# SutirthaChakraborty/RTFS-Net

Hardware: AMD Instinct MI355X
Metric: mixtures/sec forward (2 s@16 kHz, 2-spk) RTFS-Net-4 (higher is better)
Workload: dtype f32 (f16x3 split-precision MFMA products, f32 accumulate; every tensor in HBM is f32)

## Files before the change

rtfs-net_amd/csrc/api.hip:

```cpp
#include "api_common.h"
#include <atomic>
#include <vector>

namespace {

struct Cursor {
    const float* p;
    size_t off = 0;
    explicit Cursor(const float* base) : p(base) {}
    const float* take(size_t n) {
        const float* r = p ? p + off : nullptr;
        off += (n + 63) / 64 * 64;
        return r;
    }
};

struct Fork {
    hipStream_t st = nullptr;
    RtfsSide side{};
    bool open = false;
    int begin(hipStream_t owner, int slot) {
        st = owner;
        CHECK(rtfs_side_stream(owner, slot, &side));
        if (hipEventRecord(side.fork, st) != hipSuccess || hipStreamWaitEvent(side.stream, side.fork, 0) != hipSuccess) return RTFS_ERR_LAUNCH;
// ... 198 lines not shown
    a.w16_ct = reinterpret_cast<const half8*>(p.w16_ct);
    a.wf_l0 = reinterpret_cast<const half8*>(p.wf_l0);
    a.wf_l = reinterpret_cast<const half8*>(p.wf_l);
    a.wf_ct = reinterpret_cast<const half8*>(p.wf_ct);
    a.wc16 = p.wc16;
    a.bias16 = p.bias16;
    a.bt = p.bt;
    return a;
}

int dualpath(const DpPack& p, const float* x, float* out, int B, int T, int F, int dim, float* tA, float* tB, hipStream_t st) {
    const size_t plane = (size_t)T * F;
    if (dim == 4) {
        RTFS_RETURN_IF(F < 8 || F > 250, RTFS_ERR_SHAPE);
        if (!gemm_f32() && !p.whh) return launch_dualpath16(dp16_args(p, x, out, B * T, T, F, CH * plane, F, plane), st);
        return launch_dualpath(dp_args(p, x, out, T, F, CH * plane, F, plane), B * T, st);
    }
    RTFS_RETURN_IF(T < 8 || T > (p.whh ? 250 : 512), RTFS_ERR_SHAPE);
    CHECK(launch_transpose(x, tA, B * CH, T, F, st));
    if (T > 256 && !p.whh) {
        const int nb = (int)std::min<size_t>((size_t)B, (((size_t)1 << 32) - 1) / (CH * plane * sizeof(float)));
        for (int b0 = 0; b0 < B; b0 += nb) {
            const int n = std::min(nb, B - b0);
            CHECK(launch_dualpath16(dp16_args(p, tA + (size_t)b0 * CH * plane, tB + (size_t)b0 * CH * plane, n * F, F, T, CH * plane, T, plane), st));
        }
    } else if ((!gemm_f32() || T > 250) && !p.whh) {
        CHECK(launch_dualpath16(dp16_args(p, tA, tB, B * F, F, T, CH * plane, T, plane), st));
    } else {
        CHECK(launch_dualpath(dp_args(p, tA, tB, F, T, CH * plane, T, plane), B * F, st));
    }
    return launch_transpose(tB, out, B * CH, F, T, st);
}

int attention(const AttnPack& p, const float* x, float* out, int B, int T, float* q, float* k, float* v, float* o, hipStream_t st) {
    RowCanArgs a;
    a.x = x;
    a.wt = p.qkv_wt;
    a.bias = p.qkv_b;
    a.slope = p.qkv_slope;
    a.gamma = p.qkv_gamma;
    a.beta = p.qkv_beta;
    a.ngroups = 12;
    for (int g = 0; g <= 12; ++g) a.group_start[g] = g <= 8 ? 4 * g : 32 + 16 * (g - 8);
    for (int g = 0; g < 12; ++g)
        for (int o_ = a.group_start[g]; o_ < a.group_start[g + 1]; ++o_) a.group_of[o_] = (unsigned char)g;
    a.T = T;
    a.q = q;
    a.k = k;
    a.v = v;
    CHECK(launch_row_can_qkv(a, B, st));
    AttnArgs c;
    c.q = q;
    c.k = k;
    c.v = v;
    c.out = o;
    c.T = T;
    c.scale = 1.0f / 16.0f;
    CHECK(launch_attn_core(c, B, st));
    RowCanArgs r;
    r.x = o;
    r.wt = p.proj_wt;
    r.bias = p.proj_b;
    r.slope = p.proj_slope;
    r.gamma = p.proj_gamma;
    r.beta = p.proj_beta;
    r.ngroups = 1;
    r.group_start[0] = 0;
    r.group_start[1] = 64;
    r.T = T;
    r.res = x;
    r.out = out;
    return launch_row_can_proj(r, B, st);
}

struct BlockWs {
    float *residual, *x_enc, *c0, *xf0, *expanded;
    float *c1, *p0, *g, *gF, *tA, *tB, *gT, *gA, *q, *k, *v, *o;
    float *E0, *G0, *E1, *G1, *L1, *xf1, *E2, *G2;
    double* stats;
    int Bfull = 0;
    int cs = 0;
    static constexpr int NSTAT = 11;
    enum { S_C0, S_C1, S_E0, S_G0, S_E1, S_G1, S_L1, S_E2, S_G2, S_L0, S_L2 };
    BlockWs(Arena& a, int B, int T, int F, int cs_ = 0) {
        const size_t Pg = (size_t)(T / 2) * (F / 2);
        cs = cs_ ? cs_ : T * F;
        const size_t P = (size_t)cs;
        Bfull = B;
        residual = a.take<float>(B * CA * P);
        x_enc = a.take<float>(B * CH * P);
        c0 = a.take<float>(B * CH * P);
        xf0 = a.take<float>(B * CH * P);
        expanded = a.take<float>(B * CH * P);
        float** gs[] = {&c1, &p0, &g, &gF, &tA, &tB, &gT, &gA, &v, &o, &E0, &G0, &E1, &G1, &L1, &xf1, &E2, &G2};
        for (float** s : gs) *s = a.take<float>(B * CH * Pg);
        q = a.take<float>(B * CH * Pg / 4);
        k = a.take<float>(B * CH * Pg / 4);
        stats = a.take<double>((size_t)NSTAT * B * 2);
    }
    double* st(int slot, int ) const { return stats ? stats + (size_t)slot * Bfull * 2 : nullptr; }
};

int block_head(const BlockPack& p, const float* x, const float* x_res, int B, int T, int F, BlockWs& w, hipStream_t st, const CafArgs* caf, unsigned* ctr = nullptr) {
// ... 35 lines not shown
    if (zero_stats && hipMemsetAsync(w.stats, 0, sizeof(double) * W::NSTAT * w.Bfull * 2, st) != hipSuccess) return RTFS_ERR_LAUNCH;
    {
        DwArgs a;
        a.x = w.x_enc;
        a.w[0] = p.ds0_w;
        a.bias[0] = p.ds0_b;
        a.out[0] = w.c0;
        a.stats_out[0] = w.st(W::S_C0, B);
        a.C = CH; a.H = T; a.W = F; a.TH = TH_A; a.cs = w.cs;
        CHECK(launch_dw_s1(a, 1, false, 0, B, st));
    }
    DwArgs s14;
    s14.x = w.c0;
    s14.in_stats = w.st(W::S_C0, B); s14.in_inv_count = icF; s14.in_gamma = p.ds0_g; s14.in_beta = p.ds0_be;
    s14.C = CH; s14.H = T; s14.W = F; s14.TH = 64; s14.Hg = Tp; s14.Wg = Fp; s14.cs = w.cs;
    s14.w[0] = p.fus0.loc_w;
    s14.stats_out[0] = w.st(W::S_L0, B);
    s14.rev = 1;
    DwArgs s3;
    s3.x = w.c0;
    s3.in_stats = w.st(W::S_C0, B); s3.in_inv_count = icF; s3.in_gamma = p.ds0_g; s3.in_beta = p.ds0_be;
    s3.w[0] = p.ds1_w;
    s3.bias[0] = p.ds1_b;
    s3.out[0] = w.c1;
    s3.out[1] = w.p0;
    s3.stats_out[0] = w.st(W::S_C1, B);
    s3.C = CH; s3.H = T; s3.W = F; s3.Hg = Tp; s3.Wg = Fp; s3.TH = TH_C; s3.cs = w.cs;
    s3.rev = 1;
    {
        const int rc = launch_dw_s2_stats(s3, s14, B, st);
        if (rc != RTFS_OK) return rc == RTFS_ERR_ARG ? RTFS_ERR_SHAPE : rc;
    }
    CHECK(launch_g_form(w.p0, w.c1, w.st(W::S_C1, B), icG, p.ds1_g, p.ds1_be, w.g, B, CH, Pg, st));
    CHECK(dualpath(p.dpF, w.g, w.gF, B, Tp, Fp, 4, w.tA, w.tB, st));
    CHECK(dualpath(p.dpT, w.gF, w.gT, B, Tp, Fp, 3, w.tA, w.tB, st));
    CHECK(attention(p.attn, w.gT, w.gA, B, Tp, w.q, w.k, w.v, w.o, st));
    {
        DwArgs a;
        a.x = w.gA;
        a.w[0] = p.fus0.emb_w; a.w[1] = p.fus0.gate_w; a.w[2] = p.fus1.emb_w; a.w[3] = p.fus1.gate_w;
        a.out[0] = w.E0; a.out[1] = w.G0; a.out[2] = w.E1; a.out[3] = w.G1;
        a.stats_out[0] = w.st(W::S_E0, B); a.stats_out[1] = w.st(W::S_G0, B);
        a.stats_out[2] = w.st(W::S_E1, B); a.stats_out[3] = w.st(W::S_G1, B);
        a.C = CH; a.H = Tp; a.W = Fp; a.TH = TH_G;
        DwArgs l;
        l.x = w.c1;
        l.in_stats = w.st(W::S_C1, B); l.in_inv_count = icG; l.in_gamma = p.ds1_g; l.in_beta = p.ds1_be;
        l.w[0] = p.fus1.loc_w;
        l.out[0] = w.L1;
        l.stats_out[0] = w.st(W::S_L1, B);
        l.C = CH; l.H = Tp; l.W = Fp; l.TH = TH_G;
        const int rc = launch_dw_g3(a, l, B, st);
        if (rc == RTFS_ERR_ARG) {
            CHECK(launch_dw_s1(a, 4, false, 0, B, st));
            CHECK(launch_dw_s1(l, 1, true, 0, B, st));
        } else {
            CHECK(rc);
        }
    }
    {
        DwArgs a;
        a.x = w.L1; a.gate = w.G1; a.emb = w.E1;
        a.in_combine = 1;
        a.loc_stats = w.st(W::S_L1, B); a.gate_stats = w.st(W::S_G1, B); a.emb_stats = w.st(W::S_E1, B);
        a.loc_gamma = p.fus1.loc_g; a.loc_beta = p.fus1.loc_b;
        a.gate_gamma = p.fus1.gate_g; a.gate_beta = p.fus1.gate_b;
        a.emb_gamma = p.fus1.emb_g; a.emb_beta = p.fus1.emb_b;
        a.g_inv_count = icG;
        a.w[0] = p.cat0.emb_w; a.w[1] = p.cat0.gate_w;
// ... 687 lines not shown
```

rtfs-net_amd/csrc/k_attn.hip:

```cpp
#include "common.h"
#include "kernels.h"
#include "pipe_helpers.h"

#define AF 64

#define RCAN_ROWS 8
#define RCAN_LD 72
template <int NOUT>
__global__ __launch_bounds__(256, 2) void row_can_kernel(RowCanArgs a) {
    constexpr int MT = NOUT / 32, MTW = (MT + 1) / 2;
    constexpr int NR = NOUT / 4;
    constexpr float WSC = 256.f, WINV = 1.f / 256.f;
    __shared__ float Ys[NOUT][RCAN_LD];
    __shared__ float bias_s[NOUT], slope_s[NOUT];
    __shared__ float red[8];
    const int T = a.T, b = blockIdx.y;
    const int tid = threadIdx.x, lane = tid & 63, r = lane & 31, h = lane >> 5;
    const int wave = __builtin_amdgcn_readfirstlane(tid >> 6);
    const int nt = wave & 1, mp = wave >> 1;
    for (int o = tid; o < NOUT; o += 256) {
        bias_s[o] = a.bias[o] * WSC;
        slope_s[o] = a.slope[NOUT == 96 ? a.group_of[o] : 0];
    }
    half8 wh[MTW][4], wl[MTW][4];
#pragma unroll
    for (int m = 0; m < MTW; ++m) {
        const int mt = min(mp + 2 * m, MT - 1);
#pragma unroll
        for (int ks = 0; ks < 4; ++ks)
#pragma unroll
            for (int j = 0; j < 8; ++j) {
                const float w = a.wt[(ks * 16 + 8 * h + j) * NOUT + mt * 32 + r] * WSC;
                const _Float16 hi = (_Float16)w;
                wh[m][ks][j] = hi;
                wl[m][ks][j] = (_Float16)(w - (float)hi);
            }
    }
    auto ln_row = [&](int i) -> int {
        if (NOUT == 64) return wave * 16 + i;
        return i < 4 ? 4 * wave + i : i < 8 ? 16 + 4 * wave + (i - 4) : 32 + 16 * wave + (i - 8);
    };
    __shared__ float gam_s[NOUT][AF], bet_s[NOUT][AF];
    for (int i = tid; i < NOUT * AF; i += 256) {
        gam_s[0][i] = a.gamma[i];
        bet_s[0][i] = a.beta[i];
    }
    const int t0 = blockIdx.x * a.rpw;
    const int nrows = min(a.rpw, T - t0);
    const float* __restrict__ X = a.x + (size_t)b * 64 * T * AF + nt * 32 + r;
    const float* __restrict__ RES = NOUT == 64 ? a.res + ((size_t)b * 64 + wave * 16) * T * AF + lane : nullptr;
    float v[4][8];
    float rs[NOUT == 64 ? 16 : 1];
    auto load_x = [&](int t) {
#pragma unroll
        for (int ks = 0; ks < 4; ++ks)
#pragma unroll
            for (int j = 0; j < 8; ++j) v[ks][j] = X[((size_t)(ks * 16 + 8 * h + j) * T + t) * AF];
    };
    load_x(t0);
    __syncthreads();
    for (int rr = 0; rr < nrows; ++rr) {
        const int t = t0 + rr;
        half8 bh[4], bl[4];
#pragma unroll
        for (int ks = 0; ks < 4; ++ks) {
            unsigned hi[4], lo[4];
#pragma unroll
            for (int jp = 0; jp < 4; ++jp) split2(v[ks][2 * jp], v[ks][2 * jp + 1], hi[jp], lo[jp]);
            bh[ks] = __builtin_bit_cast(half8, *reinterpret_cast<f32x4*>(hi));
            bl[ks] = __builtin_bit_cast(half8, *reinterpret_cast<f32x4*>(lo));
        }
        if (NOUT == 64) {
#pragma unroll
            for (int i = 0; i < 16; ++i) rs[i] = RES[((size_t)i * T + t) * AF];
        }
        load_x(min(t + 1, T - 1));
#pragma unroll
        for (int m = 0; m < MTW; ++m) {
            const int mt = mp + 2 * m;
            if (mt < MT) {
                f32x16 acc;
#pragma unroll
                for (int q = 0; q < 16; ++q) acc[q] = bias_s[mt * 32 + (q & 3) + 8 * (q >> 2) + 4 * h];
#pragma unroll
                for (int ks = 0; ks < 4; ++ks) {
                    acc = __builtin_amdgcn_mfma_f32_32x32x16_f16(wh[m][ks], bh[ks], acc, 0, 0, 0);
                    acc = __builtin_amdgcn_mfma_f32_32x32x16_f16(wh[m][ks], bl[ks], acc, 0, 0, 0);
                    acc = __builtin_amdgcn_mfma_f32_32x32x16_f16(wl[m][ks], bh[ks], acc, 0, 0, 0);
                }
#pragma unroll
                for (int q = 0; q < 16; ++q) {
                    const int o = mt * 32 + (q & 3) + 8 * (q >> 2) + 4 * h;
                    Ys[o][nt * 32 + r] = preluf_(acc[q] * WINV, slope_s[o]);
                }
            }
        }
        __syncthreads();
        float y[NR];
#pragma unroll
        for (int i = 0; i < NR; ++i) y[i] = Ys[ln_row(i)][lane];
        if (NOUT == 96) {
#pragma unroll
            for (int g = 0; g < 3; ++g) {
                const int i0 = g == 0 ? 0 : g == 1 ? 4 : 8, gs = g == 2 ? 16 : 4;
                float s = 0.f;
#pragma unroll
                for (int i = 0; i < gs; ++i) s += y[i0 + i];
                const float mean = wave_sum(s) / (float)(gs * AF);
                float vv = 0.f;
#pragma unroll
                for (int i = 0; i < gs; ++i) {
                    y[i0 + i] -= mean;
                    vv = fmaf(y[i0 + i], y[i0 + i], vv);
                }
                const float rstd = 1.0f / sqrtf(wave_sum(vv) / (float)(gs * AF) + RTFS_EPS);
                float* __restrict__ dst = (g == 0 ? a.q : g == 1 ? a.k : a.v) + (((size_t)b * 4 + wave) * T + t) * (gs * AF) + lane;
#pragma unroll
                for (int i = 0; i < gs; ++i) dst[i * AF] = fmaf(y[i0 + i] * rstd, gam_s[ln_row(i0 + i)][lane], bet_s[ln_row(i0 + i)][lane]);
            }
        } else {
            float s = 0.f;
#pragma unroll
            for (int i = 0; i < 16; ++i) s += y[i];
            s = wave_sum(s);
            if (lane == 0) red[wave] = s;
            __syncthreads();
            const float mean = (red[0] + red[1] + red[2] + red[3]) / (float)(64 * AF);
            float vv = 0.f;
#pragma unroll
            for (int i = 0; i < 16; ++i) {
                y[i] -= mean;
                vv = fmaf(y[i], y[i], vv);
            }
            vv = wave_sum(vv);
            if (lane == 0) red[4 + wave] = vv;
            __syncthreads();
            const float rstd = 1.0f / sqrtf((red[4] + red[5] + red[6] + red[7]) / (float)(64 * AF) + RTFS_EPS);
            float* __restrict__ O = a.out + ((size_t)b * 64 + wave * 16) * T * AF + lane;
#pragma unroll
            for (int i = 0; i < 16; ++i) O[((size_t)i * T + t) * AF] = fmaf(y[i] * rstd, gam_s[ln_row(i)][lane], bet_s[ln_row(i)][lane]) + rs[i];
        }
        __syncthreads();
    }
}

#define ATT_PSC 4096.f
__device__ __forceinline__ void split8(const float (&v)[8], float sc, half8& hi, half8& lo) {
    unsigned h[4], l[4];
#pragma unroll
    for (int jp = 0; jp < 4; ++jp) split2(v[2 * jp] * sc, v[2 * jp + 1] * sc, h[jp], l[jp]);
    hi = __builtin_bit_cast(half8, *reinterpret_cast<f32x4*>(h));
    lo = __builtin_bit_cast(half8, *reinterpret_cast<f32x4*>(l));
}
__global__ __launch_bounds__(256) void attn_core_kernel(AttnArgs a) {
    extern __shared__ __attribute__((aligned(16))) float S[];
    const int T = a.T;
    const int NKT = (T + 31) >> 5;
    const int NK = NKT * 32;
    const int ldp = NK + 4;
    const int tid = threadIdx.x, lane = tid & 63, r = lane & 31, h = lane >> 5;
    const int wave = __builtin_amdgcn_readfirstlane(tid >> 6);
    const int nqt = (T + 31) >> 5;
    const int slot = blockIdx.x >> 3;
    const int pair = (slot / nqt) * 8 + (blockIdx.x & 7);
    if (pair >= a.npairs) return;
    const int q0 = (slot % nqt) * 32, hd = pair & 3, b = pair >> 2;
    const float* __restrict__ Q = a.q + ((size_t)b * 4 + hd) * T * 256;
    const float* __restrict__ K = a.k + ((size_t)b * 4 + hd) * T * 256;
    const float* __restrict__ V = a.v + ((size_t)b * 4 + hd) * T * 1024;

    for (int kg = 0; kg < NKT; kg += 8) {
// ... 89 lines not shown
        for (int ks = 0; ks < nks; ks += 2) {
            load_v(ks + 1, vv[1]);
            step(ks, vv[0]);
            load_v(min(ks + 2, nks - 1), vv[0]);
            step(ks + 1, vv[1]);
        }
        {
            const int c = col0 >> 6, f = col0 & 63;
#pragma unroll
            for (int q = 0; q < 16; ++q) {
                const int qq = q0 + (q & 3) + 8 * (q >> 2) + 4 * h;
                if (qq < T)
                    *reinterpret_cast<f32x4*>(a.out + (((size_t)b * 64 + hd * 16 + c) * T + qq) * AF + f) =
                        f32x4{o[0][q], o[1][q], o[2][q], o[3][q]} * (1.f / ATT_PSC);
            }
        }
    }
}

size_t attn_core_lds_bytes(int T) {
    const int NK = ((T + 31) >> 5) * 32;
    return (size_t)32 * (NK + 4) * sizeof(float);
}

static int rcan_rows(int T, int B) {
    if ((long)T * B >= 3500) return RCAN_ROWS;
    const int r = (int)((long)T * B / 512);
    return r < 1 ? 1 : (r > RCAN_ROWS ? RCAN_ROWS : r);
}
int launch_row_can_qkv(const RowCanArgs& a_, int B, hipStream_t st) {
    RowCanArgs a = a_;
    a.rpw = rcan_rows(a.T, B);
    if (a.ngroups != 12 || a.group_start[8] != 32 || a.group_start[12] != 96) return RTFS_ERR_SHAPE;
    hipLaunchKernelGGL(row_can_kernel<96>, dim3(cdiv(a.T, a.rpw), B), dim3(256), 0, st, a);
    return rtfs_launch_status();
}
int launch_row_can_proj(const RowCanArgs& a_, int B, hipStream_t st) {
    RowCanArgs a = a_;
    a.rpw = rcan_rows(a.T, B);
    if (a.ngroups != 1) return RTFS_ERR_SHAPE;
    hipLaunchKernelGGL(row_can_kernel<64>, dim3(cdiv(a.T, a.rpw), B), dim3(256), 0, st, a);
    return rtfs_launch_status();
}
int launch_attn_core(const AttnArgs& a, int B, hipStream_t st) {
    if (a.T < 1 || a.T > 512) return RTFS_ERR_SHAPE;
    const size_t lds = attn_core_lds_bytes(a.T);
    if (rtfs_set_max_lds((const void*)attn_core_kernel, lds) != RTFS_OK) return RTFS_ERR_LAUNCH;
    AttnArgs a2 = a;
    a2.npairs = B * 4;
    hipLaunchKernelGGL(attn_core_kernel, dim3(cdiv(a2.npairs, 8) * 8 * cdiv(a.T, 32)), dim3(256), lds, st, a2);
    return rtfs_launch_status();
}
```

rtfs-net_amd/csrc/k_dualpath16.hip:

```cpp
#include "common.h"
#include "kernels.h"
#include <stdlib.h>
#include <type_traits>


#define HLD 72
#define WLD 40
#define CLD 72
#define WINV (1.0f / 256.0f)

namespace {

__device__ __forceinline__ void split8(const float (&v)[8], half8& hi, half8& lo) {
#pragma unroll
    for (int i = 0; i < 8; ++i) {
        const _Float16 hh = (_Float16)v[i];
        hi[i] = hh;
        lo[i] = (_Float16)(v[i] - (float)hh);
    }
}

__device__ __forceinline__ float sig2(float z) { return __builtin_amdgcn_rcpf(1.0f + __builtin_amdgcn_exp2f(z)); }

__device__ __forceinline__ float take_half(float v, int ph) {
// ... 322 lines not shown
                        const int co = cot * 32 + (q & 3) + 8 * (q >> 2) + 4 * h;
                        a.out[base + (size_t)co * a.cstride + p] = fmaf(acc[t][q], WINV, res[t][q]);
                    }
                }
            }
        }
        stamp();
    }
}

size_t dp16_lds_bytes(int Ls, int nseq_per_wg) {
    return (size_t)2 * nseq_per_wg * (Ls + 1) * HLD * 2 + (size_t)2 * 2 * 256 * WLD * 2 + (size_t)nseq_per_wg * 2 * 32 * 4;
}

template <int NSEQ, int NHALF, bool PAIRED>
static int launch_dp16_stamp_t(const Dp16Args& a, hipStream_t st) {
    const size_t lds = dp16_lds_bytes(a.Ls, NSEQ);
    if (hipFuncSetAttribute((const void*)dp16_kernel<NSEQ, NHALF, PAIRED, true>, hipFuncAttributeMaxDynamicSharedMemorySize, (int)lds) != hipSuccess)
        return RTFS_ERR_LAUNCH;
    hipLaunchKernelGGL((dp16_kernel<NSEQ, NHALF, PAIRED, true>), dim3(cdiv(a.nseq, NSEQ)), dim3(512), lds, st, a);
    return rtfs_launch_status();
}

template <int NSEQ, int NHALF, bool PAIRED>
static int launch_dp16_t(const Dp16Args& a, hipStream_t st) {
    const size_t lds = dp16_lds_bytes(a.Ls, NSEQ);
    if (rtfs_set_max_lds((const void*)dp16_kernel<NSEQ, NHALF, PAIRED>, lds) != RTFS_OK) return RTFS_ERR_LAUNCH;
    void* slot = dualpath_timing_begin(a.Ls, a.nseq, st);
    hipLaunchKernelGGL((dp16_kernel<NSEQ, NHALF, PAIRED>), dim3(cdiv(a.nseq, NSEQ)), dim3(512), lds, st, a);
    dualpath_timing_end(slot, st);
    return rtfs_launch_status();
}

int launch_dualpath16(const Dp16Args& a, hipStream_t st) {
    const int L = a.Ls - 7;
    if (L < 1 || a.Ls > 512) return RTFS_ERR_SHAPE;
    static const bool gen2 = getenv("RTFS_SWEEP_GEN2") != nullptr;
    if (!gen2 || a.Ls > 256) {
        const int rc = launch_dualpath16s(a, st);
        if (rc != RTFS_ERR_SHAPE) return rc;
    }
    if (a.Ls > 256) return RTFS_ERR_SHAPE;
    if (a.stamps) {
        if (a.Ls <= 64) return launch_dp16_stamp_t<4, 2, true>(a, st);
        if (a.Ls <= 128) return launch_dp16_stamp_t<2, 4, true>(a, st);
        return launch_dp16_stamp_t<1, 4, false>(a, st);
    }
    if (a.Ls <= 64) return launch_dp16_t<4, 2, true>(a, st);
    if (a.Ls <= 128) return launch_dp16_t<2, 4, true>(a, st);
    return launch_dp16_t<1, 4, false>(a, st);
}
```

rtfs-net_amd/csrc/k_dualpath16s.hip:

```cpp
#include "common.h"
#include "kernels.h"
#include <stdlib.h>
#include <type_traits>

#define HLD 136
#define HLO 64
#define PADR 8
#define WBUF 16384
#define WINV (1.0f / 256.0f)
#ifndef DP16S_SGB
#define DP16S_SGB 1
#endif
#ifndef DP16S_WBG
#define DP16S_WBG 4
#endif
#ifndef DP16S_SGB_CT
#define DP16S_SGB_CT 1
#endif

namespace {

__device__ __forceinline__ void split8(const float (&v)[8], half8& hi, half8& lo) {
#pragma unroll
    for (int i = 0; i < 8; ++i) {
        const _Float16 hh = (_Float16)v[i];
        hi[i] = hh;
        unsigned lb;
        asm("v_fma_mixlo_f16 %0, %1, 1.0, -%2 op_sel_hi:[0,0,1]" : "=v"(lb) : "v"(v[i]), "v"(hh));
        lo[i] = __builtin_bit_cast(_Float16, (unsigned short)lb);
    }
}

__device__ __forceinline__ float ldo(const float* __restrict__ base, unsigned boff) {
    asm volatile("" : "+v"(boff));
    return *reinterpret_cast<const float*>(reinterpret_cast<const char*>(base) + boff);
}
__device__ __forceinline__ void sto(float* __restrict__ base, unsigned boff, float v) {
    asm volatile("" : "+v"(boff));
    *reinterpret_cast<float*>(reinterpret_cast<char*>(base) + boff) = v;
}

__device__ __forceinline__ float sig2(float z) { return __builtin_amdgcn_rcpf(1.0f + __builtin_amdgcn_exp2f(z)); }

__device__ __forceinline__ float take_half(float v, int ph) {
    const auto r = __builtin_amdgcn_permlane32_swap(__float_as_uint(v), __float_as_uint(v), false, false);
    return __uint_as_float(ph == 0 ? r[0] : r[1]);
}
__device__ __forceinline__ float sum_halves(float v) {
    const auto r = __builtin_amdgcn_permlane32_swap(__float_as_uint(v), __float_as_uint(v), false, false);
    return __uint_as_float(r[0]) + __uint_as_float(r[1]);
}

}

template <int NSEQ, bool PAIRED, int NT, bool STAMP = false, int NP = 4 / NT, int NPASS = 1>
__global__ __launch_bounds__(128 * NP, NT == 2 ? 2 : 4) void dp16s_kernel(Dp16Args a) {
    static_assert((NSEQ == 2 && PAIRED) || (NSEQ == 1 && !PAIRED), "F sweep: one sequence pair; T sweep: one sequence");
    static_assert(NT == 1 || NT == 2, "row tiles per wave");
    static_assert(NP == 2 || NP == 4, "time parts");
    static_assert(NPASS == 1 || (NPASS == 2 && NSEQ == 1 && NT == 2 && NP == 4), "two passes: the 4 s program only");
    constexpr int STEPS = (PAIRED ? 16 : 32) * NT;
    constexpr int NPART = NP;
    constexpr int NTHR = 128 * NPART;
    constexpr int NPIECE = 1024 / NTHR;
    constexpr int PSTEPS = STEPS * NPART;
    constexpr bool WB1 = NPASS > 1;
    extern __shared__ __attribute__((aligned(1024))) unsigned char smem[];
    const int Ls = a.Ls, L = Ls - 7, rowsH = Ls + 1 + PADR;
    half8* Wst = reinterpret_cast<half8*>(smem);
    _Float16* Hh = reinterpret_cast<_Float16*>(smem + (WB1 ? 1 : 2) * WBUF) + PADR * HLD;
    _Float16* Hl = Hh + HLO;
    float* chand = reinterpret_cast<float*>(Hh + (NSEQ * rowsH - PADR) * HLD);

    const int tid = threadIdx.x, lane = tid & 63;
    const int wave = __builtin_amdgcn_readfirstlane(tid >> 6);
    const int r = lane & 31, h = lane >> 5;
    const int part = wave >> 1, dir = wave & 1;
    const int seq = PAIRED ? h : 0;
    constexpr int CPART = PAIRED ? NPART / 2 : NPART;
    const int cseq = wave / (2 * CPART), ccot = (wave / CPART) & 1, cpart = wave % CPART;
    const int n0 = blockIdx.x * NSEQ;

    int nstamp = 0;
    auto stamp = [&]() {
        if (STAMP) {
            __builtin_amdgcn_sched_barrier(0);
            const unsigned long long t = __builtin_amdgcn_s_memtime();
            __builtin_amdgcn_s_waitcnt(0xC07F);
            if (tid == 0 && nstamp < 16) a.stamps[(size_t)blockIdx.x * 16 + nstamp] = t;
            ++nstamp;
            __builtin_amdgcn_sched_barrier(0);
        }
    };
    auto stamp_at = [&](int slot) {
        if (STAMP) {
            __builtin_amdgcn_sched_barrier(0);
            const unsigned long long t = __builtin_amdgcn_s_memtime();
            __builtin_amdgcn_s_waitcnt(0xC07F);
            if (tid == 0) a.stamps[(size_t)blockIdx.x * 16 + slot] = t;
            __builtin_amdgcn_sched_barrier(0);
        }
    };
    stamp();
    auto seq_base = [&](int s) {
        int n = n0 + s;
        n = n < a.nseq ? n : a.nseq - 1;
        return (size_t)(n / a.R) * a.bstride + (size_t)(n % a.R) * a.rstride;
    };

    half8 pre[2][NPIECE];
    auto stage_load = [&](auto set_c, const half8* __restrict__ step) {
        constexpr int S = decltype(set_c)::value;
#pragma unroll
        for (int j = 0; j < NPIECE; ++j) pre[S][j] = step[tid + NTHR * j];
    };
    auto stage_write = [&](auto set_c, int buf) {
        constexpr int S = decltype(set_c)::value;
#pragma unroll
        for (int j = 0; j < NPIECE; ++j) Wst[(WB1 ? 0 : buf) * 1024 + tid + NTHR * j] = pre[S][j];
    };
    const std::integral_constant<int, 0> S0;
    const std::integral_constant<int, 1> S1;
    stage_load(S0, a.wf_l0);

#pragma unroll 1
    for (int rb = 0; rb < NPASS; ++rb)
    if (rb * (NTHR / 2) + wave * 32 < NSEQ * Ls) {
        const int task = rb * (NTHR / 2) + wave * 32 + r, ntask = NSEQ * Ls;
        const bool live = task < ntask;
        const int tk = live ? task : ntask - 1;
        const int s = (NSEQ == 2 && tk >= Ls) ? 1 : 0, pos = tk - s * Ls;
        const unsigned xoff = (unsigned)(seq_base(s) + pos + (size_t)(32 * h) * a.cstride) * 4u;
        float v[32];
#pragma unroll
        for (int c = 0; c < 32; ++c) v[c] = ldo(a.x + (size_t)c * a.cstride, xoff);
        float sum = 0.f;
#pragma unroll
        for (int c = 0; c < 32; ++c) sum += v[c];
        const float mean = sum_halves(sum) * (1.0f / 64);
        float var = 0.f;
#pragma unroll
        for (int c = 0; c < 32; ++c) {
            const float d = v[c] - mean;
            var = fmaf(d, d, var);
        }
        const float rstd = 1.0f / sqrtf(sum_halves(var) * (1.0f / 64) + RTFS_EPS);
        _Float16* dh = Hh + (s * rowsH + pos) * HLD + 32 * h;
        _Float16* dl = Hl + (s * rowsH + pos) * HLD + 32 * h;
        if (live) {
#pragma unroll
            for (int c8 = 0; c8 < 4; ++c8) {
                float y[8];
#pragma unroll
                for (int i = 0; i < 8; ++i) y[i] = fmaf((v[c8 * 8 + i] - mean) * rstd, a.ln_gamma[32 * h + c8 * 8 + i], a.ln_beta[32 * h + c8 * 8 + i]);
                half8 hi, lo;
                split8(y, hi, lo);
                *reinterpret_cast<half8*>(dh + c8 * 8) = hi;
                *reinterpret_cast<half8*>(dl + c8 * 8) = lo;
            }
        }
        if (tid < NSEQ * 16) {
            half8 z;
#pragma unroll
            for (int i = 0; i < 8; ++i) z[i] = (_Float16)0.f;
            const int zs = tid / 16, pc = tid % 16;
            *reinterpret_cast<half8*>(Hh + (zs * rowsH + Ls) * HLD + pc * 8) = z;
        }
    }
// ... 317 lines not shown
                                    }
                                    const int k = TSTEP * t + q4 + i;
                                    char* const o = Hb + base + (BW ? KMAX - k : k) * ROWB;
                                    *reinterpret_cast<_Float16*>(o) = hh[i];
                                    *reinterpret_cast<unsigned short*>(o + HLO * 2) = (unsigned short)lo[i];
                                }
                            }
                            __builtin_amdgcn_sched_barrier(0);
                        }
                    }
                };
                if (dir)
                    wb(std::true_type());
                else
                    wb(std::false_type());
            }
        }
        if (layer == 1) stamp_at(15);
        __syncthreads();
        stamp();
        }
    };
    do_layer(0, std::true_type());
    for (int layer = 1; layer < 4; ++layer) do_layer(layer, std::false_type());

#pragma unroll 1
    for (int cp = 0; cp < NPASS; ++cp) {
        f32x16 acc[NT];
#pragma unroll
        for (int t = 0; t < NT; ++t)
#pragma unroll
            for (int q = 0; q < 16; ++q) acc[t][q] = 0.f;
        float res[NT][16];
        const size_t rbase = seq_base(cseq) + (size_t)(ccot * 32) * a.cstride;
        unsigned eoff[NT];
#pragma unroll
        for (int t = 0; t < NT; ++t) eoff[t] = (unsigned)(rbase + (size_t)(4 * h) * a.cstride + min(PSTEPS * cp + 32 * NT * cpart + 32 * t + r, Ls - 1)) * 4u;
#pragma unroll
        for (int q = 0; q < 16; ++q) {
            const int cq = (q & 3) + 8 * (q >> 2);
            const float btq = a.bt[ccot * 32 + cq + 4 * h];
#pragma unroll
            for (int t = 0; t < NT; ++t) res[t][q] = ldo(a.x + (size_t)cq * a.cstride, eoff[t]) + btq;
        }
        __builtin_amdgcn_sched_barrier(0);
        auto tap = [&](int q, auto set_c) {
            int hrow[NT];
#pragma unroll
            for (int t = 0; t < NT; ++t) {
                const int p = PSTEPS * cp + 32 * NT * cpart + 32 * t + r - q;
                hrow[t] = (cseq * rowsH + ((p >= 0 && p < L) ? p : Ls)) * HLD + 8 * h;
            }
            const half8* wb = Wst + (WB1 ? 0 : (g & 1)) * 1024 + ccot * 512 + lane;
            half8 xh[4][NT], xl[4][NT], wh[4], wl[4];
#pragma unroll
            for (int k2 = 0; k2 < 4; k2 += 2) {
#pragma unroll
                for (int kk = k2; kk < k2 + 2; ++kk) wh[kk] = wb[kk * 128];
#pragma unroll
                for (int kk = k2; kk < k2 + 2; ++kk)
#pragma unroll
                    for (int t = 0; t < NT; ++t) xh[kk][t] = *reinterpret_cast<const half8*>(Hh + hrow[t] + kk * 16);
#pragma unroll
                for (int kk = k2; kk < k2 + 2; ++kk) wl[kk] = wb[kk * 128 + 64];
#pragma unroll
                for (int kk = k2; kk < k2 + 2; ++kk)
#pragma unroll
                    for (int t = 0; t < NT; ++t) xl[kk][t] = *reinterpret_cast<const half8*>(Hl + hrow[t] + kk * 16);
            }
            if (WB1) __syncthreads();
            stage_write(set_c, (g + 1) & 1);
#pragma unroll
            for (int k2 = 0; k2 < 4; k2 += 2) {
#pragma unroll
                for (int term = 0; term < 3; ++term) {
#pragma unroll
// ... 2 lines not shown
                        for (int t = 0; t < NT; ++t)
                            acc[t] = __builtin_amdgcn_mfma_f32_32x32x16_f16(term == 1 ? wl[kk] : wh[kk], term == 2 ? xl[kk][t] : xh[kk][t], acc[t], 0, 0, 0);
                }
            }
            stage_load(set_c, a.wf_ct + (size_t)(min(8 * cp + q + 3, 8 * NPASS - 1) & 7) * 1024);
            if (NT == 2 && DP16S_SGB_CT && !WB1) {
                __builtin_amdgcn_sched_group_barrier(0x100, 6, 0);
#pragma unroll
                for (int i = 0; i < 18; ++i) {
                    __builtin_amdgcn_sched_group_barrier(0x008, 1, 0);
                    __builtin_amdgcn_sched_group_barrier(0x100, 1, 0);
                    if (i >= 14) __builtin_amdgcn_sched_group_barrier(0x200, 1, 0);
                }
#pragma unroll
                for (int i = 0; i < 4; ++i) {
                    __builtin_amdgcn_sched_group_barrier(0x008, 1, 0);
                    __builtin_amdgcn_sched_group_barrier(0x020, 1, 0);
                }
                __builtin_amdgcn_sched_group_barrier(0x008, 2, 0);
            }
            __syncthreads();
            ++g;
        };
        for (int q = 0; q < 8; q += 2) {
            tap(q, S0);
            tap(q + 1, S1);
        }
        stamp();
        if (n0 + cseq < a.nseq) {
#pragma unroll
            for (int t = 0; t < NT; ++t) {
                const int p = PSTEPS * cp + 32 * NT * cpart + 32 * t + r;
                if (p < Ls) {
#pragma unroll
                    for (int q = 0; q < 16; ++q)
                        sto(a.out + (size_t)((q & 3) + 8 * (q >> 2)) * a.cstride, eoff[t], fmaf(acc[t][q], WINV, res[t][q]));
                }
            }
        }
        stamp();
    }
}

size_t dp16s_lds_bytes(int Ls, int nseq_per_wg) {
    return (size_t)(Ls > 256 ? 1 : 2) * WBUF + (size_t)nseq_per_wg * (Ls + 1 + PADR) * HLD * 2 + (size_t)nseq_per_wg * 2 * 32 * 4;
}

template <int NSEQ, bool PAIRED, int NT, int NP = 4 / NT, int NPASS = 1>
static int launch_dp16s_t(const Dp16Args& a, hipStream_t st) {
    const size_t lds = dp16s_lds_bytes(a.Ls, NSEQ);
    constexpr bool LONG = NT == 2 && NP == 4;
    if (lds > (LONG ? 160 : 80) * 1024) return RTFS_ERR_SHAPE;
    constexpr int NTHR = 128 * NP;
    if (a.stamps) {
        if (rtfs_set_max_lds((const void*)dp16s_kernel<NSEQ, PAIRED, NT, true, NP, NPASS>, lds) != RTFS_OK) return RTFS_ERR_LAUNCH;
        hipLaunchKernelGGL((dp16s_kernel<NSEQ, PAIRED, NT, true, NP, NPASS>), dim3(cdiv(a.nseq, NSEQ)), dim3(NTHR), lds, st, a);
        return rtfs_launch_status();
    }
    if (rtfs_set_max_lds((const void*)dp16s_kernel<NSEQ, PAIRED, NT, false, NP, NPASS>, lds) != RTFS_OK) return RTFS_ERR_LAUNCH;
    void* slot = dualpath_timing_begin(a.Ls, a.nseq, st);
    hipLaunchKernelGGL((dp16s_kernel<NSEQ, PAIRED, NT, false, NP, NPASS>), dim3(cdiv(a.nseq, NSEQ)), dim3(NTHR), lds, st, a);
    dualpath_timing_end(slot, st);
    return rtfs_launch_status();
}

int launch_dualpath16s(const Dp16Args& a0, hipStream_t st) {
    const int L = a0.Ls - 7;
    if (L < 1 || a0.Ls > 512) return RTFS_ERR_SHAPE;
    if ((((size_t)(a0.nseq - 1) / a0.R) * a0.bstride + (size_t)(a0.R - 1) * a0.rstride + 63 * a0.cstride + a0.Ls) * 4 >= ((size_t)1 << 32)) return RTFS_ERR_SHAPE;
    const Dp16Args& a = a0;
    const bool pair = a0.Ls <= 64;
    if (a0.Ls > 256) return launch_dp16s_t<1, false, 2, 4, 2>(a, st);
    if (a0.Ls > 128) return launch_dp16s_t<1, false, 2, 4>(a, st);
    return pair ? launch_dp16s_t<2, true, 2>(a, st) : launch_dp16s_t<1, false, 2>(a, st);
}
```

rtfs-net_amd/csrc/kernels.h:

```cpp
#pragma once
#include <hip/hip_runtime.h>
#include <stddef.h>
#include "common.h"

struct PwArgs {
    const float* x = nullptr;
    const float* x2 = nullptr;
    float* res_out = nullptr;
    const float* wt = nullptr;
    const void* w16 = nullptr;
    const void* w16b = nullptr;
    const float* bias = nullptr;
    const float* aux = nullptr;
    float* out = nullptr;
    const double* stats = nullptr;
    double inv_count = 0;
    const float* gamma = nullptr;
    const float* beta = nullptr;
    const float* gw = nullptr;
    const float* gb = nullptr;
    const float* slope = nullptr;
    int P = 0;
    int cs = 0;
    int cout_live = 0;
// ... 141 lines not shown
int launch_dw_s1(const DwArgs& a, int nconv, bool in_affine, int mode, int B, hipStream_t st);
int launch_dw_g3(const DwArgs& conv4, const DwArgs& aff1, int B, hipStream_t st);
int launch_dw_s2_pool(const DwArgs& a, int B, hipStream_t st);
int launch_dw_s2_stats(const DwArgs& s2, const DwArgs& stats, int B, hipStream_t st);
int launch_g_form(const float* p0, const float* c1, const double* st1, double inv_count, const float* gamma,
                  const float* beta, float* g, int B, int C, int HW, hipStream_t st);
int launch_g_combine(const GCombineArgs& a, int B, hipStream_t st);
int launch_transpose(const float* x, float* y, int N, int H, int W, hipStream_t st);
int launch_stats(const float* x, double* stats, int B, size_t N, hipStream_t st);
int launch_stats2(const float* x, double* stats, int B, size_t N, double* part, hipStream_t st);

struct DpArgs {
    const float* x = nullptr;
    float* out = nullptr;
    int R = 0, Ls = 0;
    size_t bstride = 0, rstride = 0, cstride = 0;
    const float* ln_gamma = nullptr;
    const float* ln_beta = nullptr;
    const float* W0 = nullptr;
    const float* Wl = nullptr;
    const float* wc = nullptr;
    const float* bias = nullptr;
    const float* Wt = nullptr;
    const float* bt = nullptr;
    const float* whh = nullptr;
};
size_t dualpath_lds_bytes(int Ls);
int launch_dualpath(const DpArgs& a, int nseq, hipStream_t st);
int launch_sru_standalone(const float* x, float* h, int L, int N, const float* W0, const float* Wl, const float* wc,
                          const float* bias, hipStream_t st);

struct RowCanArgs {
    const float* x = nullptr;
    const float* wt = nullptr;
    const float* bias = nullptr;
    const float* slope = nullptr;
    const float* gamma = nullptr;
    const float* beta = nullptr;
    int ngroups = 0;
    int group_start[13] = {0};
    unsigned char group_of[96] = {0};
    int T = 0;
    int rpw = 0;
    float *q = nullptr, *k = nullptr, *v = nullptr;
    const float* res = nullptr;
    float* out = nullptr;
};
struct AttnArgs {
    const float *q = nullptr, *k = nullptr, *v = nullptr;
    float* out = nullptr;
    int T = 0;
    float scale = 0.f;
    int npairs = 0;
};
int launch_row_can_qkv(const RowCanArgs& a, int B, hipStream_t st);
int launch_row_can_proj(const RowCanArgs& a, int B, hipStream_t st);
int launch_attn_core(const AttnArgs& a, int B, hipStream_t st);
size_t attn_core_lds_bytes(int T);

struct CafArgs {
    const float* audio = nullptr;
    const float* video = nullptr;
    float* out = nullptr;
    float* r_out = nullptr;
    float* att_out = nullptr;
    float *r_t = nullptr, *att_t = nullptr;
    int T = 0, F = 0, Tv = 0;
    const float *w_key = nullptr, *bn_key = nullptr;
    const float *w_val = nullptr, *bn_val = nullptr;
    const float *w_att = nullptr, *b_att = nullptr, *g_att = nullptr, *be_att = nullptr;
    const float *w_resize = nullptr, *b_resize = nullptr, *g_resize = nullptr, *be_resize = nullptr;
};
int launch_caf_video(const CafArgs& a, int B, hipStream_t st);
int launch_caf_apply(const CafArgs& a, int B, hipStream_t st);
int dualpath_timing_enable(int on);
int dualpath_timing_collect(float* ms, int* ls, int* nseq, int cap);

struct Dp16Args {
    const float* x = nullptr;
    float* out = nullptr;
    int nseq = 0, R = 0, Ls = 0;
    size_t bstride = 0, rstride = 0, cstride = 0;
    const float* ln_gamma = nullptr;
    const float* ln_beta = nullptr;
    const half8* w16_l0 = nullptr;
    const half8* w16_l = nullptr;
    const half8* w16_ct = nullptr;
    const half8 *wf_l0 = nullptr, *wf_l = nullptr, *wf_ct = nullptr;
    const float* wc16 = nullptr;
    const float* bias16 = nullptr;
    const float* bt = nullptr;
    unsigned long long* stamps = nullptr;
};
size_t dp16_lds_bytes(int Ls, int nseq_per_wg);
int launch_dualpath16(const Dp16Args& a, hipStream_t st);
size_t dp16s_lds_bytes(int Ls, int nseq_per_wg);
int launch_dualpath16s(const Dp16Args& a, hipStream_t st);
void* dualpath_timing_begin(int Ls, int nseq, hipStream_t st);
void dualpath_timing_end(void* slot, hipStream_t st);

size_t vp_lds_bytes(int Tv);
int launch_vp_block(const float* video, const float* pack, float* out, int B, int Tv, hipStream_t st);

int launch_pit_pairwise(const float* est, const float* tgt, int B, int n, int L, int kind, int zero_mean, int take_log, float* pw,
                        float* min_loss, int* perm, hipStream_t st);

size_t video_pack_floats();
size_t video_workspace_bytes(int B, int T);
int video_frontend(const float* lips, const float* pack, float* out, int B, int T, void* ws, size_t ws_bytes, hipStream_t st);

struct GemmArgs {
    const float *A = nullptr, *B = nullptr;
    float* C = nullptr;
    int lda = 0, ldb = 0, ldc = 0, M = 0, N = 0, K = 0;
    int ncb = 0, nrb = 0;
    int kchunk = 0;
    const float* bias = nullptr;
    size_t sA = 0, sB = 0, sC = 0;
};
int launch_gemm_nt(const float* A, int lda, const float* Bt, int ldb, float* C, int ldc, int M, int N, int K, int mode,
                   hipStream_t st, const float* bias = nullptr, int batch = 1, size_t sA = 0, size_t sB = 0, size_t sC = 0);
int launch_gemm_tn(const float* A, int lda, const float* B, int ldb, float* C, int ldc, int M, int N, long K, hipStream_t st, int batch = 1,
                   size_t sA = 0, size_t sB = 0, size_t sC = 0);
struct SruScanArgs {
    const float* U = nullptr;
    const float* xin = nullptr;
    const float* wc = nullptr;
    const float* bias = nullptr;
    float* h = nullptr;
    float* c = nullptr;
// ... 120 lines not shown
```

Before: 3245.

## Keep dual-path intermediates channel-last to drop transposes and vectorise loads

Adds channel-last layout modes to the dp16s dual-path kernel. The frequency sweep now writes channel-last output and the time sweep reads and writes channel-last, which removes the explicit transpose kernels around the time-path call. The attention row-can kernels get a channel-last variant that reads the input and the residual with 16-byte vector loads, staging the residual through LDS. This saves two transpose launches and their HBM traffic and turns strided scalar accesses into vector ones, at the cost of more template instantiations and some extra LDS traffic for the residual.

```diff
diff --git a/rtfs-net_amd/csrc/api.hip b/rtfs-net_amd/csrc/api.hip
--- a/rtfs-net_amd/csrc/api.hip
+++ b/rtfs-net_amd/csrc/api.hip
@@ -254,9 +254,10 @@
     return launch_transpose(tB, out, B * CH, F, T, st);
 }
 
-int attention(const AttnPack& p, const float* x, float* out, int B, int T, float* q, float* k, float* v, float* o, hipStream_t st) {
+int attention(const AttnPack& p, const float* x, float* out, int B, int T, float* q, float* k, float* v, float* o, hipStream_t st, bool cl = false) {
     RowCanArgs a;
     a.x = x;
+    a.cl = cl;
     a.wt = p.qkv_wt;
     a.bias = p.qkv_b;
     a.slope = p.qkv_slope;
@@ -291,6 +292,7 @@
     r.group_start[1] = 64;
     r.T = T;
     r.res = x;
+    r.cl = cl;
     r.out = out;
     return launch_row_can_proj(r, B, st);
 }
@@ -392,9 +394,32 @@
         if (rc != RTFS_OK) return rc == RTFS_ERR_ARG ? RTFS_ERR_SHAPE : rc;
     }
     CHECK(launch_g_form(w.p0, w.c1, w.st(W::S_C1, B), icG, p.ds1_g, p.ds1_be, w.g, B, CH, Pg, st));
-    CHECK(dualpath(p.dpF, w.g, w.gF, B, Tp, Fp, 4, w.tA, w.tB, st));
-    CHECK(dualpath(p.dpT, w.gF, w.gT, B, Tp, Fp, 3, w.tA, w.tB, st));
-    CHECK(attention(p.attn, w.gT, w.gA, B, Tp, w.q, w.k, w.v, w.o, st));
+    const size_t per = (size_t)CH * Pg;
+    const int nb = (int)std::min<size_t>((size_t)B, (((size_t)1 << 32) - 1) / (per * sizeof(float)));
+    const bool cl = !p.dpF.whh && !p.dpT.whh && !gemm_f32() && !dualpath_gen2() && Fp >= 8 && Fp <= 64 && Tp >= 8 && Tp <= 512 &&
+                    nb >= 1 && (nb >= B || Tp > 256);
+    if (cl) {
+        for (int b0 = 0; b0 < B; b0 += nb) {
+            const int n = std::min(nb, B - b0);
+            Dp16Args f = dp16_args(p.dpF, w.g + b0 * per, w.gF + b0 * per, n * Tp, Tp, Fp, per, Fp, Pg);
+            f.layout = 2;
+            f.obstride = per;
+            f.orstride = (size_t)Fp * CH;
+            f.opstride = CH;
+            CHECK(launch_dualpath16(f, st));
+        }
+        for (int b0 = 0; b0 < B; b0 += nb) {
+            const int n = std::min(nb, B - b0);
+            Dp16Args t = dp16_args(p.dpT, w.gF + b0 * per, w.gT + b0 * per, n * Fp, Fp, Tp, per, CH, 1);
+            t.layout = 3;
+            t.pstride = (size_t)Fp * CH;
+            CHECK(launch_dualpath16(t, st));
+        }
+    } else {
+        CHECK(dualpath(p.dpF, w.g, w.gF, B, Tp, Fp, 4, w.tA, w.tB, st));
+        CHECK(dualpath(p.dpT, w.gF, w.gT, B, Tp, Fp, 3, w.tA, w.tB, st));
+    }
+    CHECK(attention(p.attn, w.gT, w.gA, B, Tp, w.q, w.k, w.v, w.o, st, cl));
     {
         DwArgs a;
         a.x = w.gA;
diff --git a/rtfs-net_amd/csrc/k_attn.hip b/rtfs-net_amd/csrc/k_attn.hip
--- a/rtfs-net_amd/csrc/k_attn.hip
+++ b/rtfs-net_amd/csrc/k_attn.hip
@@ -6,7 +6,7 @@
 
 #define RCAN_ROWS 8
 #define RCAN_LD 72
-template <int NOUT>
+template <int NOUT, bool CL = false>
 __global__ __launch_bounds__(256, 2) void row_can_kernel(RowCanArgs a) {
     constexpr int MT = NOUT / 32, MTW = (MT + 1) / 2;
     constexpr int NR = NOUT / 4;
@@ -14,6 +14,8 @@
     __shared__ float Ys[NOUT][RCAN_LD];
     __shared__ float bias_s[NOUT], slope_s[NOUT];
     __shared__ float red[8];
+    constexpr bool XCL = CL && NOUT == 96, RCL = CL && NOUT == 64;
+    __shared__ __attribute__((aligned(16))) float Rs[RCL ? AF : 1][RCL ? 68 : 4];
     const int T = a.T, b = blockIdx.y;
     const int tid = threadIdx.x, lane = tid & 63, r = lane & 31, h = lane >> 5;
     const int wave = __builtin_amdgcn_readfirstlane(tid >> 6);
@@ -47,15 +49,24 @@
     }
     const int t0 = blockIdx.x * a.rpw;
     const int nrows = min(a.rpw, T - t0);
-    const float* __restrict__ X = a.x + (size_t)b * 64 * T * AF + nt * 32 + r;
-    const float* __restrict__ RES = NOUT == 64 ? a.res + ((size_t)b * 64 + wave * 16) * T * AF + lane : nullptr;
+    const float* __restrict__ X = XCL ? a.x + ((size_t)b * T * AF + nt * 32 + r) * 64 + 8 * h : a.x + (size_t)b * 64 * T * AF + nt * 32 + r;
+    const float* __restrict__ RES = NOUT == 64 ? (RCL ? a.res + (size_t)b * T * AF * 64 + 4 * tid : a.res + ((size_t)b * 64 + wave * 16) * T * AF + lane)
+                                               : nullptr;
     float v[4][8];
     float rs[NOUT == 64 ? 16 : 1];
     auto load_x = [&](int t) {
-#pragma unroll
-        for (int ks = 0; ks < 4; ++ks)
-#pragma unroll
-            for (int j = 0; j < 8; ++j) v[ks][j] = X[((size_t)(ks * 16 + 8 * h + j) * T + t) * AF];
+        if constexpr (XCL) {
+#pragma unroll
+            for (int ks = 0; ks < 4; ++ks) {
+                *reinterpret_cast<f32x4*>(&v[ks][0]) = *reinterpret_cast<const f32x4*>(X + (size_t)t * AF * 64 + ks * 16);
+                *reinterpret_cast<f32x4*>(&v[ks][4]) = *reinterpret_cast<const f32x4*>(X + (size_t)t * AF * 64 + ks * 16 + 4);
+            }
+        } else {
+#pragma unroll
+            for (int ks = 0; ks < 4; ++ks)
+#pragma unroll
+                for (int j = 0; j < 8; ++j) v[ks][j] = X[((size_t)(ks * 16 + 8 * h + j) * T + t) * AF];
+        }
     };
     load_x(t0);
     __syncthreads();
@@ -70,7 +81,10 @@
             bh[ks] = __builtin_bit_cast(half8, *reinterpret_cast<f32x4*>(hi));
             bl[ks] = __builtin_bit_cast(half8, *reinterpret_cast<f32x4*>(lo));
         }
-        if (NOUT == 64) {
+        if constexpr (RCL) {
+#pragma unroll
+            for (int k = 0; k < 4; ++k) *reinterpret_cast<f32x4*>(&rs[4 * k]) = *reinterpret_cast<const f32x4*>(RES + (size_t)t * AF * 64 + 1024 * k);
+        } else if (NOUT == 64) {
 #pragma unroll
             for (int i = 0; i < 16; ++i) rs[i] = RES[((size_t)i * T + t) * AF];
         }
@@ -94,6 +108,10 @@
                     Ys[o][nt * 32 + r] = preluf_(acc[q] * WINV, slope_s[o]);
                 }
             }
+        }
+        if constexpr (RCL) {
+#pragma unroll
+            for (int k = 0; k < 4; ++k) *reinterpret_cast<f32x4*>(&Rs[tid / 16 + 16 * k][4 * (tid % 16)]) = *reinterpret_cast<const f32x4*>(&rs[4 * k]);
         }
         __syncthreads();
         float y[NR];
@@ -137,6 +155,10 @@
             __syncthreads();
             const float rstd = 1.0f / sqrtf((red[4] + red[5] + red[6] + red[7]) / (float)(64 * AF) + RTFS_EPS);
             float* __restrict__ O = a.out + ((size_t)b * 64 + wave * 16) * T * AF + lane;
+            if constexpr (RCL) {
+#pragma unroll
+                for (int k = 0; k < 4; ++k) *reinterpret_cast<f32x4*>(&rs[4 * k]) = *reinterpret_cast<const f32x4*>(&Rs[lane][wave * 16 + 4 * k]);
+            }
 #pragma unroll
             for (int i = 0; i < 16; ++i) O[((size_t)i * T + t) * AF] = fmaf(y[i] * rstd, gam_s[ln_row(i)][lane], bet_s[ln_row(i)][lane]) + rs[i];
         }
@@ -292,14 +314,20 @@
     RowCanArgs a = a_;
     a.rpw = rcan_rows(a.T, B);
     if (a.ngroups != 12 || a.group_start[8] != 32 || a.group_start[12] != 96) return RTFS_ERR_SHAPE;
-    hipLaunchKernelGGL(row_can_kernel<96>, dim3(cdiv(a.T, a.rpw), B), dim3(256), 0, st, a);
+    if (a.cl)
+        hipLaunchKernelGGL((row_can_kernel<96, true>), dim3(cdiv(a.T, a.rpw), B), dim3(256), 0, st, a);
+    else
+        hipLaunchKernelGGL((row_can_kernel<96, false>), dim3(cdiv(a.T, a.rpw), B), dim3(256), 0, st, a);
     return rtfs_launch_status();
 }
 int launch_row_can_proj(const RowCanArgs& a_, int B, hipStream_t st) {
     RowCanArgs a = a_;
     a.rpw = rcan_rows(a.T, B);
     if (a.ngroups != 1) return RTFS_ERR_SHAPE;
-    hipLaunchKernelGGL(row_can_kernel<64>, dim3(cdiv(a.T, a.rpw), B), dim3(256), 0, st, a);
+    if (a.cl)
+        hipLaunchKernelGGL((row_can_kernel<64, true>), dim3(cdiv(a.T, a.rpw), B), dim3(256), 0, st, a);
+    else
+        hipLaunchKernelGGL((row_can_kernel<64, false>), dim3(cdiv(a.T, a.rpw), B), dim3(256), 0, st, a);
     return rtfs_launch_status();
 }
 int launch_attn_core(const AttnArgs& a, int B, hipStream_t st) {
diff --git a/rtfs-net_amd/csrc/k_dualpath16.hip b/rtfs-net_amd/csrc/k_dualpath16.hip
--- a/rtfs-net_amd/csrc/k_dualpath16.hip
+++ b/rtfs-net_amd/csrc/k_dualpath16.hip
@@ -378,11 +378,16 @@
     return rtfs_launch_status();
 }
 
+bool dualpath_gen2() {
+    static const bool gen2 = getenv("RTFS_SWEEP_GEN2") != nullptr;
+    return gen2;
+}
+
 int launch_dualpath16(const Dp16Args& a, hipStream_t st) {
     const int L = a.Ls - 7;
     if (L < 1 || a.Ls > 512) return RTFS_ERR_SHAPE;
-    static const bool gen2 = getenv("RTFS_SWEEP_GEN2") != nullptr;
-    if (!gen2 || a.Ls > 256) {
+    if (a.layout != 0) return launch_dualpath16s(a, st);
+    if (!dualpath_gen2() || a.Ls > 256) {
         const int rc = launch_dualpath16s(a, st);
         if (rc != RTFS_ERR_SHAPE) return rc;
     }
diff --git a/rtfs-net_amd/csrc/k_dualpath16s.hip b/rtfs-net_amd/csrc/k_dualpath16s.hip
--- a/rtfs-net_amd/csrc/k_dualpath16s.hip
+++ b/rtfs-net_amd/csrc/k_dualpath16s.hip
@@ -39,6 +39,14 @@
     asm volatile("" : "+v"(boff));
     *reinterpret_cast<float*>(reinterpret_cast<char*>(base) + boff) = v;
 }
+__device__ __forceinline__ f32x4 ldo4(const float* __restrict__ base, unsigned boff, unsigned imm) {
+    asm volatile("" : "+v"(boff));
+    return *reinterpret_cast<const f32x4*>(reinterpret_cast<const char*>(base) + boff + imm);
+}
+__device__ __forceinline__ void sto4(float* __restrict__ base, unsigned boff, unsigned imm, f32x4 v) {
+    asm volatile("" : "+v"(boff));
+    *reinterpret_cast<f32x4*>(reinterpret_cast<char*>(base) + boff + imm) = v;
+}
 
 __device__ __forceinline__ float sig2(float z) { return __builtin_amdgcn_rcpf(1.0f + __builtin_amdgcn_exp2f(z)); }
 
@@ -53,9 +61,11 @@
 
 }
 
-template <int NSEQ, bool PAIRED, int NT, bool STAMP = false, int NP = 4 / NT, int NPASS = 1>
+template <int NSEQ, bool PAIRED, int NT, bool STAMP = false, int NP = 4 / NT, int NPASS = 1, int LAY = 0>
 __global__ __launch_bounds__(128 * NP, NT == 2 ? 2 : 4) void dp16s_kernel(Dp16Args a) {
     static_assert((NSEQ == 2 && PAIRED) || (NSEQ == 1 && !PAIRED), "F sweep: one sequence pair; T sweep: one sequence");
+    static_assert(LAY == 0 || LAY == 2 || LAY == 3, "layouts: channel-major, channel-major -> channel-last, channel-last");
+    constexpr bool XCL = LAY & 1, OCL = LAY >> 1;
     static_assert(NT == 1 || NT == 2, "row tiles per wave");
     static_assert(NP == 2 || NP == 4, "time parts");
     static_assert(NPASS == 1 || (NPASS == 2 && NSEQ == 1 && NT == 2 && NP == 4), "two passes: the 4 s program only");
@@ -107,6 +117,12 @@
         n = n < a.nseq ? n : a.nseq - 1;
         return (size_t)(n / a.R) * a.bstride + (size_t)(n % a.R) * a.rstride;
     };
+    auto out_seq_base = [&](int s) {
+        int n = n0 + s;
+        n = n < a.nseq ? n : a.nseq - 1;
+        return XCL == OCL ? (size_t)(n / a.R) * a.bstride + (size_t)(n % a.R) * a.rstride
+                          : (size_t)(n / a.R) * a.obstride + (size_t)(n % a.R) * a.orstride;
+    };
 
     half8 pre[2][NPIECE];
     auto stage_load = [&](auto set_c, const half8* __restrict__ step) {
@@ -130,10 +146,20 @@
         const bool live = task < ntask;
         const int tk = live ? task : ntask - 1;
         const int s = (NSEQ == 2 && tk >= Ls) ? 1 : 0, pos = tk - s * Ls;
-        const unsigned xoff = (unsigned)(seq_base(s) + pos + (size_t)(32 * h) * a.cstride) * 4u;
         float v[32];
-#pragma unroll
-        for (int c = 0; c < 32; ++c) v[c] = ldo(a.x + (size_t)c * a.cstride, xoff);
+        if constexpr (XCL) {
+            const unsigned xoff = (unsigned)(seq_base(s) + (size_t)pos * a.pstride + 32 * h) * 4u;
+#pragma unroll
+            for (int c4 = 0; c4 < 8; ++c4) {
+                const f32x4 q = ldo4(a.x, xoff, 16 * c4);
+#pragma unroll
+                for (int i = 0; i < 4; ++i) v[4 * c4 + i] = q[i];
+            }
+        } else {
+            const unsigned xoff = (unsigned)(seq_base(s) + pos + (size_t)(32 * h) * a.cstride) * 4u;
+#pragma unroll
+            for (int c = 0; c < 32; ++c) v[c] = ldo(a.x + (size_t)c * a.cstride, xoff);
+        }
         float sum = 0.f;
 #pragma unroll
         for (int c = 0; c < 32; ++c) sum += v[c];
@@ -517,16 +543,30 @@
 #pragma unroll
             for (int q = 0; q < 16; ++q) acc[t][q] = 0.f;
         float res[NT][16];
-        const size_t rbase = seq_base(cseq) + (size_t)(ccot * 32) * a.cstride;
         unsigned eoff[NT];
 #pragma unroll
-        for (int t = 0; t < NT; ++t) eoff[t] = (unsigned)(rbase + (size_t)(4 * h) * a.cstride + min(PSTEPS * cp + 32 * NT * cpart + 32 * t + r, Ls - 1)) * 4u;
+        for (int t = 0; t < NT; ++t) {
+            const size_t p = min(PSTEPS * cp + 32 * NT * cpart + 32 * t + r, Ls - 1);
+            eoff[t] = XCL ? (unsigned)(seq_base(cseq) + p * a.pstride + ccot * 32 + 4 * h) * 4u
+                          : (unsigned)(seq_base(cseq) + (size_t)(ccot * 32) * a.cstride + (size_t)(4 * h) * a.cstride + p) * 4u;
+        }
 #pragma unroll
         for (int q = 0; q < 16; ++q) {
             const int cq = (q & 3) + 8 * (q >> 2);
             const float btq = a.bt[ccot * 32 + cq + 4 * h];
 #pragma unroll
-            for (int t = 0; t < NT; ++t) res[t][q] = ldo(a.x + (size_t)cq * a.cstride, eoff[t]) + btq;
+            for (int t = 0; t < NT; ++t) {
+                if constexpr (XCL) {
+                    if ((q & 3) == 0) {
+                        const f32x4 x4 = ldo4(a.x, eoff[t], 32 * (q >> 2));
+#pragma unroll
+                        for (int i = 0; i < 4; ++i) res[t][q + i] = x4[i];
+                    }
+                    res[t][q] += btq;
+                } else {
+                    res[t][q] = ldo(a.x + (size_t)cq * a.cstride, eoff[t]) + btq;
+                }
+            }
         }
         __builtin_amdgcn_sched_barrier(0);
         auto tap = [&](int q, auto set_c) {
@@ -595,9 +635,20 @@
             for (int t = 0; t < NT; ++t) {
                 const int p = PSTEPS * cp + 32 * NT * cpart + 32 * t + r;
                 if (p < Ls) {
-#pragma unroll
-                    for (int q = 0; q < 16; ++q)
-                        sto(a.out + (size_t)((q & 3) + 8 * (q >> 2)) * a.cstride, eoff[t], fmaf(acc[t][q], WINV, res[t][q]));
+                    if constexpr (OCL) {
+                        const unsigned ooff = XCL ? eoff[t] : (unsigned)(out_seq_base(cseq) + (size_t)p * a.opstride + ccot * 32 + 4 * h) * 4u;
+#pragma unroll
+                        for (int j = 0; j < 4; ++j) {
+                            f32x4 y;
+#pragma unroll
+                            for (int i = 0; i < 4; ++i) y[i] = fmaf(acc[t][4 * j + i], WINV, res[t][4 * j + i]);
+                            sto4(a.out, ooff, 32 * j, y);
+                        }
+                    } else {
+#pragma unroll
+                        for (int q = 0; q < 16; ++q)
+                            sto(a.out + (size_t)((q & 3) + 8 * (q >> 2)) * a.cstride, eoff[t], fmaf(acc[t][q], WINV, res[t][q]));
+                    }
                 }
             }
         }
@@ -609,31 +660,42 @@
     return (size_t)(Ls > 256 ? 1 : 2) * WBUF + (size_t)nseq_per_wg * (Ls + 1 + PADR) * HLD * 2 + (size_t)nseq_per_wg * 2 * 32 * 4;
 }
 
-template <int NSEQ, bool PAIRED, int NT, int NP = 4 / NT, int NPASS = 1>
+template <int NSEQ, bool PAIRED, int NT, int NP = 4 / NT, int NPASS = 1, int LAY = 0>
 static int launch_dp16s_t(const Dp16Args& a, hipStream_t st) {
     const size_t lds = dp16s_lds_bytes(a.Ls, NSEQ);
     constexpr bool LONG = NT == 2 && NP == 4;
     if (lds > (LONG ? 160 : 80) * 1024) return RTFS_ERR_SHAPE;
     constexpr int NTHR = 128 * NP;
     if (a.stamps) {
+        if (LAY != 0) return RTFS_ERR_ARG;
         if (rtfs_set_max_lds((const void*)dp16s_kernel<NSEQ, PAIRED, NT, true, NP, NPASS>, lds) != RTFS_OK) return RTFS_ERR_LAUNCH;
         hipLaunchKernelGGL((dp16s_kernel<NSEQ, PAIRED, NT, true, NP, NPASS>), dim3(cdiv(a.nseq, NSEQ)), dim3(NTHR), lds, st, a);
         return rtfs_launch_status();
     }
-    if (rtfs_set_max_lds((const void*)dp16s_kernel<NSEQ, PAIRED, NT, false, NP, NPASS>, lds) != RTFS_OK) return RTFS_ERR_LAUNCH;
+    if (rtfs_set_max_lds((const void*)dp16s_kernel<NSEQ, PAIRED, NT, false, NP, NPASS, LAY>, lds) != RTFS_OK) return RTFS_ERR_LAUNCH;
     void* slot = dualpath_timing_begin(a.Ls, a.nseq, st);
-    hipLaunchKernelGGL((dp16s_kernel<NSEQ, PAIRED, NT, false, NP, NPASS>), dim3(cdiv(a.nseq, NSEQ)), dim3(NTHR), lds, st, a);
+    hipLaunchKernelGGL((dp16s_kernel<NSEQ, PAIRED, NT, false, NP, NPASS, LAY>), dim3(cdiv(a.nseq, NSEQ)), dim3(NTHR), lds, st, a);
     dualpath_timing_end(slot, st);
     return rtfs_launch_status();
 }
 
-int launch_dualpath16s(const Dp16Args& a0, hipStream_t st) {
-    const int L = a0.Ls - 7;
-    if (L < 1 || a0.Ls > 512) return RTFS_ERR_SHAPE;
-    if ((((size_t)(a0.nseq - 1) / a0.R) * a0.bstride + (size_t)(a0.R - 1) * a0.rstride + 63 * a0.cstride + a0.Ls) * 4 >= ((size_t)1 << 32)) return RTFS_ERR_SHAPE;
-    const Dp16Args& a = a0;
-    const bool pair = a0.Ls <= 64;
-    if (a0.Ls > 256) return launch_dp16s_t<1, false, 2, 4, 2>(a, st);
-    if (a0.Ls > 128) return launch_dp16s_t<1, false, 2, 4>(a, st);
-    return pair ? launch_dp16s_t<2, true, 2>(a, st) : launch_dp16s_t<1, false, 2>(a, st);
-}
+template <int LAY>
+static int launch_dp16s_lay(const Dp16Args& a, hipStream_t st) {
+    if (a.Ls > 256) return launch_dp16s_t<1, false, 2, 4, 2, LAY>(a, st);
+    if (a.Ls > 128) return launch_dp16s_t<1, false, 2, 4, 1, LAY>(a, st);
+    return a.Ls <= 64 ? launch_dp16s_t<2, true, 2, 2, 1, LAY>(a, st) : launch_dp16s_t<1, false, 2, 2, 1, LAY>(a, st);
+}
+
+int launch_dualpath16s(const Dp16Args& a, hipStream_t st) {
+    const int L = a.Ls - 7;
+    if (L < 1 || a.Ls > 512) return RTFS_ERR_SHAPE;
+    if (a.layout != 0 && a.layout != 2 && a.layout != 3) return RTFS_ERR_ARG;
+    const bool xcl = a.layout & 1, ocl = a.layout >> 1;
+    const size_t nb = (size_t)(a.nseq - 1) / a.R, nr = (size_t)(a.R - 1), lp = (size_t)(a.Ls - 1);
+    const size_t xspan = nb * a.bstride + nr * a.rstride + (xcl ? lp * a.pstride + 63 : 63 * a.cstride + lp);
+    const size_t ospan = xcl == ocl ? xspan : nb * a.obstride + nr * a.orstride + lp * a.opstride + 63;
+    if ((std::max(xspan, ospan) + 1) * 4 >= ((size_t)1 << 32)) return RTFS_ERR_SHAPE;
+    if (a.layout == 3) return launch_dp16s_lay<3>(a, st);
+    if (a.layout == 2) return launch_dp16s_lay<2>(a, st);
+    return launch_dp16s_lay<0>(a, st);
+}
diff --git a/rtfs-net_amd/csrc/kernels.h b/rtfs-net_amd/csrc/kernels.h
--- a/rtfs-net_amd/csrc/kernels.h
+++ b/rtfs-net_amd/csrc/kernels.h
@@ -197,6 +197,7 @@
 
 struct RowCanArgs {
     const float* x = nullptr;
+    int cl = 0;
     const float* wt = nullptr;
     const float* bias = nullptr;
     const float* slope = nullptr;
@@ -246,6 +247,9 @@
     float* out = nullptr;
     int nseq = 0, R = 0, Ls = 0;
     size_t bstride = 0, rstride = 0, cstride = 0;
+    int layout = 0;
+    size_t pstride = 0;
+    size_t obstride = 0, orstride = 0, opstride = 0;
     const float* ln_gamma = nullptr;
     const float* ln_beta = nullptr;
     const half8* w16_l0 = nullptr;
@@ -261,6 +265,7 @@
 int launch_dualpath16(const Dp16Args& a, hipStream_t st);
 size_t dp16s_lds_bytes(int Ls, int nseq_per_wg);
 int launch_dualpath16s(const Dp16Args& a, hipStream_t st);
+bool dualpath_gen2();
 void* dualpath_timing_begin(int Ls, int nseq, hipStream_t st);
 void dualpath_timing_end(void* slot, hipStream_t st);
 
```

After: 3311 (median of 6 runs). +2.0%, better.
